# wienkers/marEx

Measured on AMD Instinct MI355X. Metric: Mcells*timesteps/s, shifting_baseline + hobday_extreme p95 (validation+anomaly+thresholds+mask), higher is better.
Workload: dtype f32

## Files before the change

### marex_amd/csrc/marex_common.hip.h

```cpp
#pragma once
#include <hip/hip_runtime.h>

#include <cmath>
#include <type_traits>
#include <cstdarg>
#include <cstdio>
#include <cstring>
#include <map>
#include <string>
#include <vector>

#include "marex_hip.h"

#define NDOY MAREX_NDOY

struct TimedLaunch {
    int kid;
    hipEvent_t a, b;
};

struct marex_ctx {
    int device = 0;
    hipStream_t stream = nullptr;
    std::string err;
    bool timing = false;
    std::vector<TimedLaunch> pending;
    double total_ms[MAREX_K_COUNT] = {0};
    int64_t launches[MAREX_K_COUNT] = {0};
    int* shift_info = nullptr;
    int* shift_plan = nullptr;
    size_t shift_plan_years = 0;
    int* shift_lplan = nullptr;
    size_t shift_lplan_years = 0;
    unsigned char* thr_scratch = nullptr;
    size_t thr_scratch_bytes = 0;
    unsigned char* detrend_scratch = nullptr;
    size_t detrend_scratch_bytes = 0;
    unsigned char* morph_scratch = nullptr;
    size_t morph_scratch_bytes = 0;
    int n_cu = 0;
    std::map<std::string, int> opts;
    long long* row_off = nullptr;
    size_t row_off_bytes = 0;
    long long* row_off_mask = nullptr;
    size_t row_off_mask_bytes = 0;
    unsigned long long* dbg_counters = nullptr;
};

#define MAREX_DBG_COUNTERS 8

static inline int ctx_opt(marex_ctx* ctx, const char* name, int dflt) {
    auto it = ctx->opts.find(name);
    return it == ctx->opts.end() ? dflt : it->second;
}

#ifdef MAREX_ABLATION
#define MAREX_ABLATE_OPT(ctx, name) ctx_opt(ctx, name, 0)
#else
#define MAREX_ABLATE_OPT(ctx, name) 0
#endif

static inline unsigned long long* ctx_debug_counters(marex_ctx* ctx) {
    if (!ctx->dbg_counters) {
        if (hipMalloc((void**)&ctx->dbg_counters, MAREX_DBG_COUNTERS * sizeof(unsigned long long)) != hipSuccess) return nullptr;
        (void)hipMemsetAsync(ctx->dbg_counters, 0, MAREX_DBG_COUNTERS * sizeof(unsigned long long), ctx->stream);
    }
    return ctx->dbg_counters;
}

static inline int device_cus(marex_ctx* ctx) {
    if (ctx->n_cu <= 0) {
        int n = 0;
        if (hipDeviceGetAttribute(&n, hipDeviceAttributeMultiprocessorCount, ctx->device) != hipSuccess || n <= 0) n = 256;
        ctx->n_cu = n;
    }
    return ctx->n_cu;
}

static inline int fail(marex_ctx* ctx, int code, const char* fmt, ...) {
    char buf[512];
    va_list ap;
    va_start(ap, fmt);
    vsnprintf(buf, sizeof buf, fmt, ap);
    va_end(ap);
    if (ctx) ctx->err = buf;
    return code;
}

#define HIP_TRY(ctx, expr)                                                                      \
    do {                                                                                        \
        hipError_t e__ = (expr);                                                                \
        if (e__ != hipSuccess) return fail(ctx, -2, "%s failed: %s", #expr, hipGetErrorString(e__)); \
    } while (0)

struct LaunchTimer {
    marex_ctx* ctx;
    int kid;
    hipEvent_t a = nullptr, b = nullptr;
    LaunchTimer(marex_ctx* c, int k) : ctx(c), kid(k) {
        if (ctx->timing) {
            (void)hipEventCreate(&a);
            (void)hipEventCreate(&b);
            (void)hipEventRecord(a, ctx->stream);
        }
    }
    ~LaunchTimer() {
        if (ctx->timing) {
            (void)hipEventRecord(b, ctx->stream);
            ctx->pending.push_back({kid, a, b});
        }
    }
};

static inline void drain_timers(marex_ctx* ctx) {
    for (auto& p : ctx->pending) {
        float ms = 0.f;
// ... 97 lines not shown
```

### marex_amd/csrc/marex_context.hip

```cpp
#include "marex_common.hip.h"

extern "C" int marex_abi_version(void) { return MAREX_ABI_VERSION; }

extern "C" int marex_workspace_bytes(const marex_workspace_cfg* cfg, size_t* bytes) {
    if (!cfg || !bytes || cfg->T <= 0 || cfg->T_out <= 0 || cfg->T_out > cfg->T || cfg->C <= 0) return -1;
    const size_t C = (size_t)cfg->C, To = (size_t)cfg->T_out;
    for (int i = 0; i < MAREX_WS_COUNT; ++i) bytes[i] = 0;
    bytes[MAREX_WS_ANOMALY] = To * C * sizeof(float);
    bytes[MAREX_WS_EXTREME] = To * C;
    bytes[MAREX_WS_THRESHOLDS] = (size_t)MAREX_NDOY * C * sizeof(float);
    if (cfg->list_rows > 0) {
        const int nper = marex_tail_lists(cfg->max_bucket, cfg->list_rows);
        if (nper < 1) return -1;
        const size_t nch = cfg->list_rows <= 16 ? 2 : 4;
        bytes[MAREX_WS_LISTS] = (size_t)MAREX_NDOY * (size_t)nper * nch * C * 16;
        bytes[MAREX_WS_AUX] = (size_t)MAREX_NDOY * C * sizeof(uint32_t);
    } else {
        bytes[MAREX_WS_BINS] = ((C + 15) / 16) * To * 16 * sizeof(uint16_t);
    }
    bytes[MAREX_WS_PER_CELL] = C * (sizeof(uint8_t) + sizeof(int32_t));
    bytes[MAREX_WS_TOTAL] = bytes[MAREX_WS_ANOMALY] + bytes[MAREX_WS_EXTREME] + 2 * bytes[MAREX_WS_THRESHOLDS] + bytes[MAREX_WS_LISTS] +
                            bytes[MAREX_WS_AUX] + bytes[MAREX_WS_BINS] + bytes[MAREX_WS_PER_CELL];
    return 0;
}

extern "C" int marex_create(int device, marex_ctx** out) {
    if (!out) return -1;
    int n = 0;
    if (hipGetDeviceCount(&n) != hipSuccess || device < 0 || device >= n) return -3;
    marex_ctx* c = new marex_ctx();
    c->device = device;
    extern char** environ;
    for (char** e = environ; e && *e; ++e) {
        if (strncmp(*e, "MAREX_", 6) != 0) continue;
        const char* eq = strchr(*e, '=');
        if (!eq || eq == *e + 6) continue;
        char* end = nullptr;
        const long v = strtol(eq + 1, &end, 10);
        if (end == eq + 1 || *end != '\0') continue;
        c->opts[std::string(*e + 6, (size_t)(eq - (*e + 6)))] = (int)v;
    }
    *out = c;
    return 0;
}

extern "C" int marex_set_option(marex_ctx* ctx, const char* name, int value) {
    if (!ctx || !name || !*name) return -1;
    ctx->opts[name] = value;
    return 0;
}

extern "C" int marex_clear_option(marex_ctx* ctx, const char* name) {
    if (!ctx) return -1;
    if (!name)
        ctx->opts.clear();
    else
        ctx->opts.erase(name);
    return 0;
}

extern "C" int marex_debug_counters(marex_ctx* ctx, uint64_t* out, int reset) {
    if (!ctx || !out) return -1;
    HIP_TRY(ctx, hipSetDevice(ctx->device));
    unsigned long long* d = ctx_debug_counters(ctx);
    if (!d) return fail(ctx, -2, "marex_debug_counters: allocation failed");
    HIP_TRY(ctx, hipStreamSynchronize(ctx->stream));
    HIP_TRY(ctx, hipMemcpy(out, d, MAREX_DBG_COUNTERS * sizeof(unsigned long long), hipMemcpyDeviceToHost));
    if (reset) HIP_TRY(ctx, hipMemsetAsync(d, 0, MAREX_DBG_COUNTERS * sizeof(unsigned long long), ctx->stream));
    return 0;
}

extern "C" int marex_destroy(marex_ctx* ctx) {
    if (!ctx) return -1;
    drain_timers(ctx);
    if (ctx->shift_info) (void)hipFree(ctx->shift_info);
    if (ctx->shift_plan) (void)hipFree(ctx->shift_plan);
    if (ctx->shift_lplan) (void)hipFree(ctx->shift_lplan);
    if (ctx->thr_scratch) (void)hipFree(ctx->thr_scratch);
    if (ctx->detrend_scratch) (void)hipFree(ctx->detrend_scratch);
    if (ctx->morph_scratch) (void)hipFree(ctx->morph_scratch);
    if (ctx->dbg_counters) (void)hipFree(ctx->dbg_counters);
    if (ctx->row_off) (void)hipFree(ctx->row_off);
    if (ctx->row_off_mask) (void)hipFree(ctx->row_off_mask);
    delete ctx;
    return 0;
}

extern "C" const char* marex_last_error(marex_ctx* ctx) { return ctx ? ctx->err.c_str() : "null context"; }

extern "C" int marex_set_stream(marex_ctx* ctx, void* s) {
    if (!ctx) return -1;
    ctx->stream = (hipStream_t)s;
    return 0;
}

extern "C" int marex_sync(marex_ctx* ctx) {
    if (!ctx) return -1;
    HIP_TRY(ctx, hipSetDevice(ctx->device));
    HIP_TRY(ctx, hipStreamSynchronize(ctx->stream));
    drain_timers(ctx);
    return 0;
}

extern "C" int marex_timing_enable(marex_ctx* ctx, int on) {
    if (!ctx) return -1;
    ctx->timing = on != 0;
    return 0;
}

extern "C" int marex_timing_reset(marex_ctx* ctx) {
    if (!ctx) return -1;
    drain_timers(ctx);
    memset(ctx->total_ms, 0, sizeof ctx->total_ms);
    memset(ctx->launches, 0, sizeof ctx->launches);
    return 0;
}

extern "C" int marex_timing_get(marex_ctx* ctx, int kid, double* total_ms, int64_t* launches) {
    if (!ctx || kid < 0 || kid >= MAREX_K_COUNT) return -1;
    drain_timers(ctx);
    if (total_ms) *total_ms = ctx->total_ms[kid];
    if (launches) *launches = ctx->launches[kid];
    return 0;
}
```

### marex_amd/csrc/marex_shifting.hip

```cpp
#include "marex_common.hip.h"
#include "marex_tails.hip.h"
#include <numeric>
#include <utility>

template <int D, int SCAP, bool SEXACT, int WCAP, bool RREG>
__global__ void __launch_bounds__(256)
k_shifting(const float* __restrict__ x, long T, long C, const int4* __restrict__ year_plan, int n_cal, int W,
           int S_rt, int write_clim, const float* __restrict__ edges, int nb, long T_out, float* __restrict__ out,
           unsigned short* __restrict__ bins, unsigned char* __restrict__ mask, int* __restrict__ invalid_count,
           int ncb, int nchunks, int ablate, const int* __restrict__ skip) {
    extern __shared__ float lds[];
#ifndef MAREX_ABLATION
    ablate = 0;
#endif
    float* ring = lds;
    float rr[RREG ? D : 1][RREG ? WCAP : 1];
    const int npad = WCAP - W;
    int4* lplan = reinterpret_cast<int4*>(lds + (RREG ? (size_t)0 : (size_t)D * WCAP * 256));
    float* e = reinterpret_cast<float*>(lplan + (size_t)n_cal * D);

    int cb, chunk;
    if (!xcd_swizzle(blockIdx.x, ncb, nchunks, cb, chunk)) return;
    if (D == 4 && skip && skip[chunk]) return;
    const int tid = threadIdx.x;
// ... 245 lines not shown
}
__device__ __forceinline__ v2f splat2(float v) { return (v2f){v, v}; }

__device__ __forceinline__ v2f div_const2(v2f a, float b, float y) {
    const v2f q = a * splat2(y);
    const v2f r = __builtin_elementwise_fma(-q, splat2(b), a);
    const v2f q2 = __builtin_elementwise_fma(r, splat2(y), q);
    return (v2f){__builtin_amdgcn_div_fixupf(q2.x, b, a.x), __builtin_amdgcn_div_fixupf(q2.y, b, a.y)};
}

typedef __amdgpu_buffer_rsrc_t rsrc_t;
__device__ __forceinline__ rsrc_t make_rsrc(const void* base) {
    return __builtin_amdgcn_make_buffer_rsrc(const_cast<void*>(base), 0, -1, 0x00020000);
}
__device__ __forceinline__ float ldb_f32(rsrc_t r, unsigned voff, int soff) {
    return __builtin_bit_cast(float, __builtin_amdgcn_raw_buffer_load_b32(r, (int)voff, soff, 0));
}
#ifndef ST_AUX_F32
#define ST_AUX_F32 2
#endif
#ifndef ST_AUX_U16
#define ST_AUX_U16 0
#endif
__device__ __forceinline__ void stb_f32(rsrc_t r, unsigned voff, int soff, float v) {
    __builtin_amdgcn_raw_buffer_store_b32(__builtin_bit_cast(unsigned, v), r, (int)voff, soff, ST_AUX_F32);
}
__device__ __forceinline__ void stb_u16(rsrc_t r, unsigned voff, int soff, int v) {
    __builtin_amdgcn_raw_buffer_store_b16((unsigned short)v, r, (int)voff, soff, ST_AUX_U16);
}

typedef int tl_out_rsrc_t __attribute__((ext_vector_type(4)));
__device__ __forceinline__ tl_out_rsrc_t tl_out_make_rsrc(const void* base) {
    const unsigned long long b = (unsigned long long)base;
    tl_out_rsrc_t r;
    r.x = __builtin_amdgcn_readfirstlane((int)(unsigned)b);
    r.y = __builtin_amdgcn_readfirstlane((int)((unsigned)(b >> 32) & 0xFFFFu));
    r.z = -1;
    r.w = 0x00020000;
    return r;
}
__device__ __forceinline__ void tl_out_store(tl_out_rsrc_t r, unsigned voff, unsigned soff, const unsigned (&w)[4]) {
    typedef unsigned u4 __attribute__((ext_vector_type(4)));
    const u4 v = {w[0], w[1], w[2], w[3]};
    const int soff_u = __builtin_amdgcn_readfirstlane((int)soff);
    asm volatile("buffer_store_dwordx4 %0, %1, %2, %3 offen nt\n\ts_nop 2" : : "v"(v), "v"(voff), "s"(r), "s"(soff_u) : "memory");
}


template <int RPW>
struct DmaRows;
#define MAREX_DMA_X4(m, so) "s_mov_b32 m0, " m "\n\ts_nop 0\n\tbuffer_load_dwordx4 %1, %3, " so " offen lds\n\t"
#define MAREX_DMA_X1(m, so) "s_mov_b32 m0, " m "\n\ts_nop 0\n\tbuffer_load_dword %2, %3, " so " offen lds\n\t"
template <>
struct DmaRows<9> {
    static constexpr int NL = 3;
    static __device__ __forceinline__ void issue(tl_out_rsrc_t r, unsigned voff4, unsigned voff1, unsigned l0, unsigned lstep, unsigned so0, unsigned rowb) {
        unsigned keep;
        const unsigned l1 = l0 + 4 * lstep, l2 = l0 + 8 * lstep, so1 = so0 + 4 * rowb, so2 = so0 + 8 * rowb;
        asm volatile("s_mov_b32 %0, m0\n\t" MAREX_DMA_X4("%4", "%7") MAREX_DMA_X4("%5", "%8") MAREX_DMA_X1("%6", "%9") "s_mov_b32 m0, %0"
                     : "=&s"(keep) : "v"(voff4), "v"(voff1), "s"(r), "s"(l0), "s"(l1), "s"(l2), "s"(so0), "s"(so1), "s"(so2) : "memory");
    }
};
template <>
struct DmaRows<8> {
    static constexpr int NL = 2;
    static __device__ __forceinline__ void issue(tl_out_rsrc_t r, unsigned voff4, unsigned voff1, unsigned l0, unsigned lstep, unsigned so0, unsigned rowb) {
        unsigned keep;
        const unsigned l1 = l0 + 4 * lstep, so1 = so0 + 4 * rowb;
        asm volatile("s_mov_b32 %0, m0\n\t" MAREX_DMA_X4("%4", "%6") MAREX_DMA_X4("%5", "%7") "s_mov_b32 m0, %0"
                     : "=&s"(keep) : "v"(voff4), "v"(voff1), "s"(r), "s"(l0), "s"(l1), "s"(so0), "s"(so1) : "memory");
    }
};
template <>
struct DmaRows<7> {
    static constexpr int NL = 4;
    static __device__ __forceinline__ void issue(tl_out_rsrc_t r, unsigned voff4, unsigned voff1, unsigned l0, unsigned lstep, unsigned so0, unsigned rowb) {
        unsigned keep;
        const unsigned l1 = l0 + 4 * lstep, l2 = l0 + 5 * lstep, l3 = l0 + 6 * lstep;
        const unsigned so1 = so0 + 4 * rowb, so2 = so0 + 5 * rowb, so3 = so0 + 6 * rowb;
        asm volatile("s_mov_b32 %0, m0\n\t" MAREX_DMA_X4("%4", "%8") MAREX_DMA_X1("%5", "%9") MAREX_DMA_X1("%6", "%10") MAREX_DMA_X1("%7", "%11") "s_mov_b32 m0, %0"
                     : "=&s"(keep) : "v"(voff4), "v"(voff1), "s"(r), "s"(l0), "s"(l1), "s"(l2), "s"(l3), "s"(so0), "s"(so1), "s"(so2), "s"(so3) : "memory");
    }
};
#undef MAREX_DMA_X4
#undef MAREX_DMA_X1

#define SHIFT_INFO_WORDS 128
#define CLASSIFY_SPLIT 11
#define LEAN_CHUNKS 96

__global__ void k_shift_classify(const int4* __restrict__ year_plan, int n_cal, const float* __restrict__ edges, int nb,
                                 int want_bins, int enable, int* __restrict__ info, int4* __restrict__ fplan, long T, long C,
                                 int reg_S, int4* __restrict__ lplan, const int* __restrict__ doy_start, int wpb, int lean_bins) {
    __shared__ int s_edges_ok;
    const int t = threadIdx.x;
    int eok = 1;
    if (want_bins) {
        const float first = edges[1], delta = edges[2] - edges[1];
        for (int j = 1 + t; j <= nb; j += (int)blockDim.x)
            eok = eok && __float_as_uint(edges[j]) == __float_as_uint(arange_edge(j, first, delta));
    }
    eok = __syncthreads_and(eok);
    if (t == 0) {
        int ok = eok;
        if (want_bins) {
            const float first = edges[1], delta = edges[2] - edges[1], last = edges[nb];
            ok = ok && delta > 0.f && nb < 32768;
            const double m = fabs((double)first) > fabs((double)last) ? fabs((double)first) : fabs((double)last);
            ok = ok && ((double)nb + 2.0 * m / (double)delta) * (1.0 / 1048576.0) < 1.0 / 256.0;
        }
        s_edges_ok = ok && enable;
        info[92] = s_edges_ok;
    }
    __shared__ int s_ok[92];
    if (t < 92) s_ok[t] = 1;
    __syncthreads();
    const int chunk = t / CLASSIFY_SPLIT, sub = t % CLASSIFY_SPLIT;
    if (chunk < 92) {
        const int d0 = chunk * 4;
        int ok = 1;
        for (int y = sub; y < n_cal; y += CLASSIFY_SPLIT) {
            int4 e[4];
            for (int i = 0; i < 4; ++i)
                e[i] = (d0 + i < NDOY) ? year_plan[(size_t)y * NDOY + d0 + i] : make_int4(-1, -1, -1, 0);
            int m = 0;
            while (m < 4 && e[m].x >= 0) ++m;
            if (fplan) {
                const int yn = y + 1 < n_cal ? y + 1 : n_cal - 1;
                const int tbw = year_plan[(size_t)yn * NDOY + (chunk >> 2) * 16].x;
                fplan[((size_t)y * 92 + chunk) * 2] = make_int4(e[0].x, e[0].y, m, e[0].z);
                fplan[((size_t)y * 92 + chunk) * 2 + 1] = make_int4(e[1].z, e[2].z, e[3].z, tbw);
            }
            for (int i = m; i < 4; ++i) ok = ok && e[i].x < 0;
            for (int i = 1; i < m; ++i) {
                ok = ok && e[i].x == e[0].x + i;
                if (e[0].y >= 0)
                    ok = ok && e[i].y == e[0].y + i && e[i].z >= 0;
                else
                    ok = ok && e[i].y < 0;
            }
            if (m > 0 && e[0].y >= 0) ok = ok && e[0].z >= 0;
        }
        if (!ok) atomicAnd(&s_ok[chunk], 0);
    }
    __syncthreads();
    if (chunk < 92 && lplan && reg_S > 0) {
        const int H = reg_S / 2, NPAIR = (reg_S + 3) / 2, NROWS = wpb * ((reg_S + 4 * wpb - 1 + wpb - 1) / wpb);
        const int d0 = chunk * 4, blk16 = (chunk / wpb) * wpb * 4;
        int D1 = 0, D2 = 0, D3 = 0;
        if (lean_bins && d0 + 3 < NDOY)
            for (int y2 = 0; y2 < n_cal; ++y2) {
                const int z0 = year_plan[(size_t)y2 * NDOY + d0].z, z1 = year_plan[(size_t)y2 * NDOY + d0 + 1].z;
                const int z2 = year_plan[(size_t)y2 * NDOY + d0 + 2].z, z3 = year_plan[(size_t)y2 * NDOY + d0 + 3].z;
                if (z0 >= 0 && z1 >= 0 && z2 >= 0 && z3 >= 0) {
                    D1 = z1 - z0;
                    D2 = z2 - z0;
                    D3 = z3 - z0;
                    break;
                }
            }
        for (int yy = sub - 1; yy <= n_cal; yy += CLASSIFY_SPLIT) {
            int flags = 0, tbv = -1, pos = 0;
            long long xoff = 0, ooff = 0;
            if (yy + 1 >= 0 && yy + 1 < n_cal) {
                const int tbn = year_plan[(size_t)(yy + 1) * NDOY + blk16].x;
                if (tbn >= H && (long)tbn - H + NROWS <= T) {
// ... 380 lines not shown
                        stb_u16(rbins, bin_lane, pA.w * 32, k0);
                        if (has1) stb_u16(rbins, bin_lane, pB.x * 32, k1);
                        if (has2) stb_u16(rbins, bin_lane, pB.y * 32, k2);
                        if (has3) stb_u16(rbins, bin_lane, pB.z * 32, k3);
                    }
                }
            }
        }
        rA[J + W] = smA;
        rB[J + W] = smB;
        SSTAMP(tsC);
        if (DMA) {
            if (stage_next) {
                if (dma_pf)
                    asm volatile("s_waitcnt vmcnt(%0)" ::"n"(DmaRows<RPW>::NL) : "memory");
                else
                    asm volatile("s_waitcnt vmcnt(0)" ::: "memory");
            }
            if (o_n > 0 && active) {
                const rsrc_t ro = make_rsrc(out + (size_t)pA.y * C);
                stb_f32(ro, voff, 0, oA.x);
                if (o_n > 1) stb_f32(ro, voff, rowb, oA.y);
                if (o_n > 2) stb_f32(ro, voff, 2 * rowb, oB.x);
                if (o_n > 3) stb_f32(ro, voff, 3 * rowb, oB.y);
            }
            asm volatile("s_barrier" ::: "memory");
        } else {
        if (stage_next) stage_store((y + 1) & 1, nx);
        if (!(SHIFT_EXP & 1)) __syncthreads();
        }
#ifdef SHIFT_STAMPS
        const unsigned long long tsD = __builtin_amdgcn_s_memtime();
        st_top += tsB - tsA;
        st_mid += tsC - tsB;
        st_end += tsD - tsC;
#endif
    };
    for (int y = 0; y < n_cal; y += 2) {
        one_year(y, std::integral_constant<int, 0>{});
        if (TAILS && t_slot == SHIFT_LIST) tails_flush();
        if (y + 1 < n_cal) one_year(y + 1, std::integral_constant<int, 1>{});
        if (TAILS && t_slot == SHIFT_LIST) tails_flush();
#pragma unroll
        for (int j = 0; j < W; ++j) {
            rA[j] = rA[j + 2];
            rB[j] = rB[j + 2];
        }
    }
    if (TAILS && mine) {
        if (t_slot > 0) tails_flush();
        while (t_list < tails.nper) tails_flush();
        if (active) {
            const unsigned cn[4] = {t_cntA & 0xFFFFu, t_cntA >> 16, t_cntB & 0xFFFFu, t_cntB >> 16};
            const unsigned ov[4] = {t_ovfA & 0xFFFFu, t_ovfA >> 16, t_ovfB & 0xFFFFu, t_ovfB >> 16};
#pragma unroll
            for (int di = 0; di < 4; ++di)
                if (d0 + di < NDOY) tails.aux[(size_t)(d0 + di) * C + c] = tail_aux_word(cn[di], ov[di]);
        }
    }
    if (invalid_count && active && n_invalid) atomicAdd(&invalid_count[c], n_invalid);
#ifdef SHIFT_STAMPS
    if (TAILS && lane == 0 && tails.dbg) {
        atomicAdd(&tails.dbg[5], st_top);
        atomicAdd(&tails.dbg[6], st_mid);
        atomicAdd(&tails.dbg[7], st_end);
        atomicAdd(&tails.dbg[4], 1ull);
    }
#endif
}

template <typename F, int... Is>
__device__ __forceinline__ void unroll_steps_impl(F& f, std::integer_sequence<int, Is...>) {
    (f(std::integral_constant<int, Is>{}), ...);
}
template <int N, typename F>
__device__ __forceinline__ void unroll_steps(F&& f) {
    unroll_steps_impl(f, std::make_integer_sequence<int, N>{});
}

#define LR_REG 1
#define LR_OUT 2
#define LR_STAGE_NEXT 4

template <int W, int S, int NWV, bool BINS>
__global__ void __launch_bounds__(64 * NWV, 16 / NWV)
k_shift_lean(const float* __restrict__ x, int T, int C, const int4* __restrict__ fplan, const int4* __restrict__ lplan, int n_cal,
             const int* __restrict__ info, const float* __restrict__ edges, int nb, float* __restrict__ out,
             unsigned char* __restrict__ mask, int* __restrict__ invalid_count, int ncg, int nblk, TailOut tails,
             unsigned short* __restrict__ bins, long T_out) {
    int cg, bc;
    if (!xcd_swizzle(blockIdx.x, ncg, nblk, cg, bc)) return;
    const int wave = __builtin_amdgcn_readfirstlane((int)(threadIdx.x >> 6));
    const int lane = (int)(threadIdx.x & 63);
    const int chunk = bc * NWV + wave;
    static_assert((S & 1) == 1 && S >= 5 && S <= 25, "k_shift_lean: odd smoothing widths 5..25");
    static_assert(NWV == 4 || NWV == 8, "k_shift_lean: 4 or 8 waves");
    constexpr int H = S / 2, NPAIR = (S + 3) / 2, NST = S + 4 * NWV - 1, RPW = (NST + NWV - 1) / NWV;
    constexpr int NROWS = NWV * RPW;
    __shared__ float stage[NROWS * 64];
    __shared__ unsigned newkeys[BINS ? 1 : NWV][2][BINS ? 1 : SHIFT_LIST][64];
    const bool mine = chunk < 92 && info[chunk] != 0;
    const int d0 = mine ? chunk * 4 : 0;
    const int c = cg * 64 + lane;
    const bool active = c < C;
    const unsigned cidx = active ? (unsigned)c : (unsigned)(C - 1);
    const unsigned voff = cidx * 4u;
    const int rowb = C * 4;
    const float e_first = edges[1], e_delta = edges[2] - edges[1], e_last = edges[nb];
    const float inv_width = (float)(nb - 1) / (e_last - e_first);
    constexpr float Sf = (float)S;
    const float yS = 1.0f / Sf;
    const float Wf = (float)W;
    const float yW = 1.0f / Wf;
    const float nbm1f = (float)(nb - 1);
    const float c0 = (1.0f - e_first * inv_width) - 0.0078125f;
    const float qnan = nan_f();
    if (chunk == 0 && mine && mask && active) mask[c] = finite_f(x[c]) ? 1 : 0;
    const unsigned bin_lane = (((cidx >> 4) - (unsigned)(cg * 4)) * (unsigned)T_out * 16u + (cidx & 15u)) * 2u;
    const rsrc_t rbins = make_rsrc(BINS ? bins + (size_t)(cg * 4) * (size_t)T_out * 16 : nullptr);
    int bD1 = 0, bD2 = 0, bD3 = 0;

    typedef __attribute__((address_space(3))) float lds_f32;
    const int c4 = cg * 64 + (lane & 15) * 4;
    const unsigned dma_voff4 = (unsigned)(lane >> 4) * (unsigned)rowb + (unsigned)(c4 + 4 <= C ? c4 : C - 4) * 4u;
    const unsigned dma_lds = (unsigned)__builtin_amdgcn_readfirstlane((int)(unsigned)(size_t)(lds_f32*)&stage[(RPW * wave) * 64]);
    const char* xw = reinterpret_cast<const char*>(x) + (size_t)(RPW * wave) * (size_t)C * 4;
    auto dma_rows = [&](int lo, int hi) __attribute__((always_inline)) {
        const unsigned long long off = ((unsigned long long)(unsigned)hi << 32) | (unsigned)lo;
        DmaRows<RPW>::issue(tl_out_make_rsrc(xw + off), dma_voff4, voff, dma_lds, 256u, 0u, (unsigned)rowb);
    };
    constexpr int LSTRIDE = LEAN_CHUNKS * 2;
    const int4* lr_next = lplan + (size_t)chunk * 2;
    {
        const int4 pre = lr_next[0];
        if (BINS) {
            const int4 preB = lr_next[1];
            bD1 = preB.y;
            bD2 = preB.z;
            bD3 = preB.w;
        }
        if (pre.x & LR_STAGE_NEXT) {
            dma_rows(pre.z, pre.w);
            asm volatile("s_waitcnt vmcnt(0)" ::: "memory");
        }
        asm volatile("s_barrier" ::: "memory");
        lr_next += LSTRIDE;
    }
    int4 nA = lr_next[0], nB = lr_next[1];
    lr_next += LSTRIDE;

    constexpr int U = W >= 13 ? 3 : 2;
    v2f hA[W + U], hB[W + U];
#pragma unroll
    for (int j = 0; j < W + U; ++j) hA[j] = hB[j] = splat2(qnan);
    int n_invalid = 0;
    unsigned t_cntA = 0, t_cntB = 0, t_ovfA = 0, t_ovfB = 0;
    int t_slot = 0, t_list = 0;
    int n_lean = 0, n_gen = 0;
    auto tails_flush = [&]() __attribute__((always_inline)) {
        const tl_out_rsrc_t rl = tl_out_make_rsrc(tails.lists + (size_t)d0 * tails.nper * 2 * (size_t)C);
        const unsigned lvoff = cidx * 16u;
#pragma unroll
        for (int pr = 0; pr < 2; ++pr) {
            unsigned v[16];
#pragma unroll
            for (int u = 0; u < 16; ++u) v[u] = (u < SHIFT_LIST && u < t_slot) ? newkeys[wave][pr][u][lane] : 0u;
            sort16_desc(v);
#pragma unroll
            for (int h = 0; h < 2; ++h) {
                const int di = 2 * pr + h;
                if (d0 + di < NDOY) {
#pragma unroll
                    for (int jj = 0; jj < 2; ++jj) {
                        unsigned w[4];
#pragma unroll
                        for (int i = 0; i < 4; ++i) {
                            const unsigned a = v[8 * jj + 2 * i], b = v[8 * jj + 2 * i + 1];
                            w[i] = h == 0 ? ((a & 0xFFFFu) | (b << 16)) : ((a >> 16) | (b & 0xFFFF0000u));
                        }
                        const int li = __builtin_amdgcn_readfirstlane((di * tails.nper + t_list) * 2 + jj);
                        if (active) tl_out_store(rl, lvoff, (unsigned)li * (unsigned)C * 16u, w);
                    }
                }
            }
        }
        ++t_list;
        t_slot = 0;
    };

    auto mid = [&](const int4& cA) __attribute__((always_inline)) {
        asm volatile("s_waitcnt lgkmcnt(0)\n\ts_barrier" ::: "memory");
        if (cA.x & LR_STAGE_NEXT) dma_rows(cA.z, cA.w);
        nA = lr_next[0];
        nB = lr_next[1];
        lr_next += LSTRIDE;
    };
    constexpr int NH0 = (NPAIR + 1) / 2, NH1 = NPAIR - NH0;
    static_assert(NH0 >= 2, "the second chain starts in the first half");
    v2f xh[NH0];
    v2f accA = splat2(0.f), accB = splat2(0.f);
    float xc0 = 0.f, xc1 = 0.f, xc2 = 0.f, xc3 = 0.f;
    auto load_half = [&](auto Pc, int how, int ts) __attribute__((always_inline)) {
        constexpr int P = decltype(Pc)::value, M0 = P ? NH0 : 0, MN = P ? NH1 : NH0;
        if (how == 0) {
            const float* st = &stage[(4 * wave) * 64 + lane];
#pragma unroll
            for (int m = 0; m < MN; ++m) {
                xh[m].x = st[(2 * (M0 + m)) * 64];
                xh[m].y = st[(2 * (M0 + m) + 1) * 64];
            }
        } else if (how == 1) {
            const rsrc_t rx = make_rsrc(x + (size_t)(ts - H) * (size_t)C);
#pragma unroll
            for (int m = 0; m < MN; ++m) {
                xh[m].x = ldb_f32(rx, voff, (2 * (M0 + m)) * rowb);
                xh[m].y = ldb_f32(rx, voff, (2 * (M0 + m) + 1) * rowb);
            }
        } else {
#pragma unroll
            for (int m = 0; m < MN; ++m) {
                int ra = ts - H + 2 * (M0 + m), rb = ra + 1;
                ra = ra < 0 ? 0 : (ra > T - 1 ? T - 1 : ra);
                rb = rb < 0 ? 0 : (rb > T - 1 ? T - 1 : rb);
                xh[m].x = ldb_f32(make_rsrc(x + (size_t)ra * (size_t)C), voff, 0);
                xh[m].y = ldb_f32(make_rsrc(x + (size_t)rb * (size_t)C), voff, 0);
            }
        }
    };
    auto half = [&](auto Pc) __attribute__((always_inline)) {
        constexpr int P = decltype(Pc)::value, M0 = P ? NH0 : 0, M1 = P ? NPAIR : NH0;
        if constexpr (S == 21) {
#define PK_LO(acc, src) "v_pk_add_f32 %" #acc ", %" #acc ", %" #src " op_sel_hi:[1,0]\n\t"
#define PK_HI(acc, src) "v_pk_add_f32 %" #acc ", %" #acc ", %" #src " op_sel:[0,1] op_sel_hi:[1,1]\n\t"
#define PK_BOTH(src) PK_LO(0, src) PK_LO(1, src) PK_HI(0, src) PK_HI(1, src)
            if (P == 0) {
                accA = (v2f){xh[0].x, -0.0f};
                accB = (v2f){xh[1].x, -0.0f};
                asm(PK_HI(0, 2) PK_LO(0, 3) PK_HI(0, 3) PK_HI(1, 3) PK_BOTH(4) PK_BOTH(5) PK_BOTH(6) PK_BOTH(7)
                    : "+v"(accA), "+v"(accB)
                    : "v"(xh[0]), "v"(xh[1]), "v"(xh[2]), "v"(xh[3]), "v"(xh[4]), "v"(xh[5]));
                xc0 = xh[5].x;
                xc1 = xh[5].y;
            } else {
                asm(PK_BOTH(2) PK_BOTH(3) PK_BOTH(4) PK_BOTH(5) PK_LO(0, 6) PK_LO(1, 6) PK_HI(1, 6) PK_LO(1, 7)
                    : "+v"(accA), "+v"(accB)
                    : "v"(xh[0]), "v"(xh[1]), "v"(xh[2]), "v"(xh[3]), "v"(xh[4]), "v"(xh[5]));
                accA.y += xh[4].y;
                accB.y += xh[5].y;
                xc2 = xh[0].x;
                xc3 = xh[0].y;
            }
#undef PK_BOTH
#undef PK_HI
#undef PK_LO
            return;
        }
        if (P == 0) accA = (v2f){xh[0].x, -0.0f};
#pragma unroll
        for (int s = 1; s <= S - 1; ++s)
            if ((s >> 1) >= M0 && (s >> 1) < M1) accA = (s & 1) ? pk_add_bc_hi(accA, xh[(s >> 1) - M0]) : pk_add_bc_lo(accA, xh[(s >> 1) - M0]);
        if ((S >> 1) >= M0 && (S >> 1) < M1) accA.y += xh[(S >> 1) - M0].y;
        if (1 >= M0 && 1 < M1) accB = (v2f){xh[1 - M0].x, -0.0f};
#pragma unroll
        for (int s = 3; s <= S + 1; ++s)
            if ((s >> 1) >= M0 && (s >> 1) < M1) accB = (s & 1) ? pk_add_bc_hi(accB, xh[(s >> 1) - M0]) : pk_add_bc_lo(accB, xh[(s >> 1) - M0]);
        if (((S + 2) >> 1) >= M0 && ((S + 2) >> 1) < M1) accB.y += xh[((S + 2) >> 1) - M0].y;
#define MAREX_XC(i, dst) \
    if (((H + i) >> 1) >= M0 && ((H + i) >> 1) < M1) dst = ((H + i) & 1) ? xh[((H + i) >> 1) - M0].y : xh[((H + i) >> 1) - M0].x;
        MAREX_XC(0, xc0) MAREX_XC(1, xc1) MAREX_XC(2, xc2) MAREX_XC(3, xc3)
#undef MAREX_XC
    };
    auto smooth = [&](const int4& cA, v2f& smA, v2f& smB, v2f& xcA, v2f& xcB, int how, int ts) __attribute__((always_inline)) {
        load_half(std::integral_constant<int, 0>{}, how, ts);
        half(std::integral_constant<int, 0>{});
        load_half(std::integral_constant<int, 1>{}, how, ts);
// ... 165 lines not shown
            const bool staged = tb >= H && tb - H + NROWS <= T && pA.x == tb + 4 * wave;
            v2f xcA, xcB;
            smooth(cA, smA, smB, xcA, xcB, staged ? 0 : (edge ? 2 : 1), pA.x);
            if (edge) {
                const int t0 = pA.x;
                smA.x = (t0 - H >= 0 && t0 + H < T) ? smA.x : qnan;
                smA.y = (t0 + 1 - H >= 0 && t0 + 1 + H < T) ? smA.y : qnan;
                smB.x = (t0 + 2 - H >= 0 && t0 + 2 + H < T) ? smB.x : qnan;
                smB.y = (t0 + 3 - H >= 0 && t0 + 3 + H < T) ? smB.y : qnan;
            }
            const bool has1 = nd > 1, has2 = nd > 2, has3 = nd > 3;
            n_invalid += finite_f(xcA.x) ? 0 : 1;
            if (has1) n_invalid += finite_f(xcA.y) ? 0 : 1; else smA.y = qnan;
            if (has2) n_invalid += finite_f(xcB.x) ? 0 : 1; else smB.x = qnan;
            if (has3) n_invalid += finite_f(xcB.y) ? 0 : 1; else smB.y = qnan;
            asm volatile("s_waitcnt vmcnt(0)" ::: "memory");
            if (pA.y >= 0) {
                v2f aA, aB;
                anomaly(Jc, xcA, xcB, aA, aB);
                const rsrc_t ro = make_rsrc(out + (size_t)pA.y * (size_t)C);
                if (active) {
                    stb_f32(ro, voff, 0, aA.x);
                    if (has1) stb_f32(ro, voff, rowb, aA.y);
                    if (has2) stb_f32(ro, voff, 2 * rowb, aB.x);
                    if (has3) stb_f32(ro, voff, 3 * rowb, aB.y);
                }
                int k0, k1, k2, k3;
                digit2(aA, k0, k1);
                digit2(aB, k2, k3);
                if constexpr (BINS) {
                    if (active) {
                        stb_u16(rbins, bin_lane, pA.w * 32, (aA.x == aA.x) ? k0 : nb);
                        if (has1) stb_u16(rbins, bin_lane, pB.x * 32, (aA.y == aA.y) ? k1 : nb);
                        if (has2) stb_u16(rbins, bin_lane, pB.y * 32, (aB.x == aB.x) ? k2 : nb);
                        if (has3) stb_u16(rbins, bin_lane, pB.z * 32, (aB.y == aB.y) ? k3 : nb);
                    }
                } else {
                const float l1 = has1 ? e_last : -__builtin_inff(), l2 = has2 ? e_last : -__builtin_inff(),
                            l3 = has3 ? e_last : -__builtin_inff();
                const bool v0 = aA.x < e_last, v1 = aA.y < l1, v2 = aB.x < l2, v3 = aB.y < l3;
                const int ds0 = tails.doy_start[d0], ds1 = tails.doy_start[d0 + 1 < NDOY ? d0 + 1 : NDOY - 1];
                const int ds2 = tails.doy_start[d0 + 2 < NDOY ? d0 + 2 : NDOY - 1], ds3 = tails.doy_start[d0 + 3 < NDOY ? d0 + 3 : NDOY - 1];
                const unsigned p0 = (unsigned)(pA.w - ds0), p1 = (unsigned)(pB.x - ds1), p2 = (unsigned)(pB.y - ds2), p3 = (unsigned)(pB.z - ds3);
                const unsigned q0 = v0 ? ((unsigned)k0 << TAIL_POS_BITS) + 128u + p0 : 0u, q1 = v1 ? ((unsigned)k1 << TAIL_POS_BITS) + 128u + p1 : 0u;
                const unsigned q2 = v2 ? ((unsigned)k2 << TAIL_POS_BITS) + 128u + p2 : 0u, q3 = v3 ? ((unsigned)k3 << TAIL_POS_BITS) + 128u + p3 : 0u;
                newkeys[wave][0][t_slot][lane] = q0 | (q1 << 16);
                newkeys[wave][1][t_slot][lane] = q2 | (q3 << 16);
                t_cntA += (v0 ? 1u : 0u) + (v1 ? 0x10000u : 0u);
                t_cntB += (v2 ? 1u : 0u) + (v3 ? 0x10000u : 0u);
                const float mx = fmaxf(fmaxf(aA.x, has1 ? aA.y : aA.x), fmaxf(has2 ? aB.x : aA.x, has3 ? aB.y : aA.x));
                if (__builtin_amdgcn_ballot_w64(mx >= e_last) != 0) {
                    unsigned s0 = t_ovfA & 0xFFFFu, s1 = t_ovfA >> 16, s2 = t_ovfB & 0xFFFFu, s3 = t_ovfB >> 16;
                    if (aA.x >= e_last) s0 = tail_ovf_add(s0, p0);
                    if (has1 && aA.y >= e_last) s1 = tail_ovf_add(s1, p1);
                    if (has2 && aB.x >= e_last) s2 = tail_ovf_add(s2, p2);
                    if (has3 && aB.y >= e_last) s3 = tail_ovf_add(s3, p3);
                    t_ovfA = s0 | (s1 << 16);
                    t_ovfB = s2 | (s3 << 16);
                }
                ++t_slot;
                }
            }
        } else {
            mid(cA);
            asm volatile("s_waitcnt vmcnt(0)" ::: "memory");
        }
        hA[J + W] = smA;
        hB[J + W] = smB;
    };

#define MAREX_LEAN_YEAR(J, yy)                                                                                  \
    {                                                                                                           \
        const int4 cA = nA, cB = nB;                                                                            \
        if (mine && (cA.x & LR_REG)) {                                                                          \
            lean_year(std::integral_constant<int, J>{}, cA, cB);                                                \
            ++n_lean;                                                                                           \
        } else {                                                                                                \
            general_year(std::integral_constant<int, J>{}, yy, cA);                                             \
            n_gen += mine ? 1 : 0;                                                                              \
        }                                                                                                       \
        asm volatile("s_barrier" ::: "memory");  \
        if (!BINS && t_slot == SHIFT_LIST) tails_flush();                                                       \
    }
    for (int y = 0; y < n_cal; y += U) {
        MAREX_LEAN_YEAR(0, y)
        if constexpr (U > 1) if (y + 1 < n_cal) MAREX_LEAN_YEAR(1, y + 1)
        if constexpr (U > 2) if (y + 2 < n_cal) MAREX_LEAN_YEAR(2, y + 2)
        if constexpr (U > 3) if (y + 3 < n_cal) MAREX_LEAN_YEAR(3, y + 3)
#pragma unroll
        for (int j = 0; j < W; ++j) {
            hA[j] = hA[j + U];
            hB[j] = hB[j + U];
        }
    }
#undef MAREX_LEAN_YEAR
    if (mine && !BINS) {
        if (t_slot > 0) tails_flush();
        while (t_list < tails.nper) tails_flush();
        if (active) {
            const unsigned cn[4] = {t_cntA & 0xFFFFu, t_cntA >> 16, t_cntB & 0xFFFFu, t_cntB >> 16};
            const unsigned ov[4] = {t_ovfA & 0xFFFFu, t_ovfA >> 16, t_ovfB & 0xFFFFu, t_ovfB >> 16};
#pragma unroll
            for (int di = 0; di < 4; ++di)
                if (d0 + di < NDOY) tails.aux[(size_t)(d0 + di) * (size_t)C + c] = tail_aux_word(cn[di], ov[di]);
        }
    }
    if (invalid_count && active && n_invalid) atomicAdd(&invalid_count[c], n_invalid);
#ifdef MAREX_LEAN_COUNTERS
    if (tails.dbg && lane == 0) {
        atomicAdd(&tails.dbg[6], (unsigned long long)n_lean);
        atomicAdd(&tails.dbg[7], (unsigned long long)n_gen);
    }
#endif
}

static bool lean_instance(int W, int S) { return S == 21 && (W == 15 || W == 5); }

struct ShiftArgs {
    const float* x;
    int64_t T, C;
    const int4* year_plan;
    const int4* fplan;
    int n_cal;
    int W, S, write_clim;
    const float* edges;
    int nb;
    int64_t T_out;
    float* out;
    uint16_t* bins;
    uint8_t* mask;
    int32_t* invalid_count;
    const int* skip;
    TailOut tails;
    bool lean = false;
    const int4* lplan = nullptr;
    int lean_waves = 4;
};

template <int D, int SCAP, bool SEXACT, int WCAP, bool RREG>
static int launch_shifting(marex_ctx* ctx, const ShiftArgs& a) {
    const int ncb = (int)((a.C + 255) / 256);
    const int nchunks = (NDOY + D - 1) / D;
    const size_t lds = ((RREG ? (size_t)0 : (size_t)D * WCAP * 256) + (a.bins ? (size_t)a.nb + 1 : 0)) * sizeof(float) + (size_t)a.n_cal * D * 16;
    if (lds > 80 * 1024) return fail(ctx, -4, "marex_shifting_baseline_f32: window_year_baseline=%d needs more than 80 KiB of LDS", a.W);
    auto kern = k_shifting<D, SCAP, SEXACT, WCAP, RREG>;
    if (lds > 48 * 1024)
        HIP_TRY(ctx, hipFuncSetAttribute((const void*)kern, hipFuncAttributeMaxDynamicSharedMemorySize, (int)lds));
    hipLaunchKernelGGL(kern, dim3(xcd_grid(ncb, nchunks)), dim3(256), lds, ctx->stream, a.x, (long)a.T, (long)a.C,
                       a.year_plan, a.n_cal, a.W, a.S, a.write_clim, a.edges, a.nb, (long)a.T_out, a.out, a.bins,
                       a.mask, a.invalid_count, ncb, nchunks, MAREX_ABLATE_OPT(ctx, "SHIFT_ABLATE"), D == 4 ? a.skip : nullptr);
    HIP_TRY(ctx, hipGetLastError());
    return 0;
}

template <int W, int S = 21>
static void launch_shift_fast(marex_ctx* ctx, const ShiftArgs& a) {
    const int ncg = (int)((a.C + 63) / 64);
#define MAREX_SF_ARGS dim3(xcd_grid(ncg, 23)), dim3(256), 0, ctx->stream, a.x, (long)a.T, (long)a.C, a.fplan, a.n_cal, a.skip, a.write_clim, a.edges, a.nb, (long)a.T_out, a.out, a.bins, a.mask, a.invalid_count, ncg, 23, a.tails
    if (a.lean && (a.tails.lists || a.bins)) {
        if constexpr (S == 21 && (W == 15 || W == 5)) {
            if (a.tails.lists)
                hipLaunchKernelGGL((k_shift_lean<W, S, 4, false>), dim3(xcd_grid(ncg, 23)), dim3(256), 0, ctx->stream, a.x, (int)a.T, (int)a.C,
                                   a.fplan, a.lplan, a.n_cal, a.skip, a.edges, a.nb, a.out, a.mask, a.invalid_count, ncg, 23, a.tails,
                                   (unsigned short*)nullptr, (long)a.T_out);
            else
                hipLaunchKernelGGL((k_shift_lean<W, S, 4, true>), dim3(xcd_grid(ncg, 23)), dim3(256), 0, ctx->stream, a.x, (int)a.T, (int)a.C,
                                   a.fplan, a.lplan, a.n_cal, a.skip, a.edges, a.nb, a.out, a.mask, a.invalid_count, ncg, 23, a.tails,
                                   a.bins, (long)a.T_out);
        }
    } else if (a.tails.lists) {
        constexpr int RPW = (S + 15 + 3) / 4;
        constexpr bool has_dma = S == 21 && (W == 15 || W == 5);
        const bool dma = has_dma && ctx_opt(ctx, "SHIFT_DMA", 0) != 0 && a.C >= 4 && a.C % 4 == 0 &&
                         (unsigned long long)(365 + 4 * RPW + 4) * (unsigned long long)a.C * 4ull < 0xFFFFFFFFull;
        if (dma)
            hipLaunchKernelGGL((k_shift_fast<W, true, S, has_dma>), MAREX_SF_ARGS);
        else
            hipLaunchKernelGGL((k_shift_fast<W, true, S, false>), MAREX_SF_ARGS);
    } else {
        hipLaunchKernelGGL((k_shift_fast<W, false, S, false>), MAREX_SF_ARGS);
    }
#undef MAREX_SF_ARGS
}

template <int D, int WCAP, bool RREG>
static int dispatch_shifting_S(marex_ctx* ctx, const ShiftArgs& a) {
    if (a.S == 21) return launch_shifting<D, 21, true, WCAP, RREG>(ctx, a);
    return launch_shifting<D, 1, false, WCAP, RREG>(ctx, a);
}

static int shifting_impl(marex_ctx* ctx, const char* who, const float* x, int64_t T, int64_t C, const int32_t* year_plan,
                         int n_cal_years, int W, int S, int write_clim, const float* edges, int nb, int64_t T_out, float* out,
                         uint16_t* bins, uint8_t* mask, int32_t* invalid_count, TailOut tails, bool* all_fast_possible) {
    if (!ctx) return -1;
    if (!x || !year_plan || !out || T <= 0 || C <= 0 || n_cal_years <= 0)
        return fail(ctx, -1, "%s: null pointer or empty shape", who);
    if (((uintptr_t)year_plan & 15) != 0) return fail(ctx, -1, "%s: year_plan must be 16-byte aligned", who);
    if (W < 1 || S < 1) return fail(ctx, -1, "%s: W and S must be >= 1", who);
    if (S > T) S = (int)T + 1;
    if (W > 64) return fail(ctx, -4, "%s: window_year_baseline > 64 is not supported", who);
    if ((bins || tails.lists) && (!edges || nb < 4 || nb > 65534 || T_out <= 0))
        return fail(ctx, -1, "%s: binning needs edges, T_out and 4 <= nb <= 65534", who);
    HIP_TRY(ctx, hipSetDevice(ctx->device));
    ShiftArgs a{x, T, C, reinterpret_cast<const int4*>(year_plan), nullptr, n_cal_years, W, S, write_clim,
                edges, nb, T_out, out, bins, mask, invalid_count, nullptr, tails};
    const int forceD = ctx_opt(ctx, "SHIFT_D", 0);
    const int reg = ctx_opt(ctx, "SHIFT_RING", 1);
    const bool fast_w = W == 3 || W == 4 || W == 5 || W == 6 || W == 7 || W == 10 || W == 13 || W == 15;
    const bool fast_ws = S == 21 ? fast_w : ((S == 11 || S == 15) && (W == 5 || W == 10 || W == 15));
    const bool fast_cfg = ctx_opt(ctx, "SHIFT_FAST", 1) != 0 && fast_ws && forceD == 0 && T >= S + 3 &&
                          T_out < (1 << 24) && C < (1 << 24) && MAREX_ABLATE_OPT(ctx, "SHIFT_ABLATE") == 0;
    if (all_fast_possible) *all_fast_possible = fast_cfg;
    if (fast_cfg && !ctx->shift_info) HIP_TRY(ctx, hipMalloc((void**)&ctx->shift_info, SHIFT_INFO_WORDS * sizeof(int)));
    if (fast_cfg && ctx->shift_plan_years < (size_t)n_cal_years) {
        if (ctx->shift_plan) {
            HIP_TRY(ctx, hipStreamSynchronize(ctx->stream));
            (void)hipFree(ctx->shift_plan);
            ctx->shift_plan = nullptr;
            ctx->shift_plan_years = 0;
        }
        HIP_TRY(ctx, hipMalloc((void**)&ctx->shift_plan, (size_t)n_cal_years * 92 * 8 * sizeof(int)));
        ctx->shift_plan_years = (size_t)n_cal_years;
    }
    LaunchTimer lt(ctx, MAREX_K_SHIFTING);
    if (fast_cfg) {
        const bool lean_bins = !tails.lists && bins && !write_clim && ctx_opt(ctx, "SHIFT_LEAN_BINS", 1) != 0;
        const bool lean = (tails.lists || lean_bins) && lean_instance(W, S) && ctx_opt(ctx, "SHIFT_LEAN", 1) != 0 && C >= 4 && C % 4 == 0 &&
                          T < (1ll << 31) - 64 && (unsigned long long)(S + 31 + 8 + 4) * (unsigned long long)C * 4ull < 0xFFFFFFFFull;
        const int lean_waves = 4;
        if (lean && ctx->shift_lplan_years < (size_t)n_cal_years) {
            if (ctx->shift_lplan) {
                HIP_TRY(ctx, hipStreamSynchronize(ctx->stream));
                (void)hipFree(ctx->shift_lplan);
                ctx->shift_lplan = nullptr;
                ctx->shift_lplan_years = 0;
            }
            HIP_TRY(ctx, hipMalloc((void**)&ctx->shift_lplan, ((size_t)n_cal_years + 2) * LEAN_CHUNKS * 8 * sizeof(int)));
            ctx->shift_lplan_years = (size_t)n_cal_years;
        }
        hipLaunchKernelGGL(k_shift_classify, dim3(1), dim3(1024), 0, ctx->stream, a.year_plan, n_cal_years, edges, nb,
                           (bins || tails.lists) ? 1 : 0, 1, ctx->shift_info, reinterpret_cast<int4*>(ctx->shift_plan), (long)T, (long)C,
                           lean ? S : 0, lean ? reinterpret_cast<int4*>(ctx->shift_lplan) : nullptr, tails.doy_start, lean_waves,
                           (lean && lean_bins) ? 1 : 0);
        a.lean_waves = lean_waves;
        a.lplan = reinterpret_cast<const int4*>(ctx->shift_lplan);
        a.lean = lean;
        a.skip = ctx->shift_info;
        a.fplan = reinterpret_cast<const int4*>(ctx->shift_plan);
        if (S == 11 || S == 15) {
            switch (W * 100 + S) {
                case 511: launch_shift_fast<5, 11>(ctx, a); break;
                case 515: launch_shift_fast<5, 15>(ctx, a); break;
                case 1011: launch_shift_fast<10, 11>(ctx, a); break;
                case 1015: launch_shift_fast<10, 15>(ctx, a); break;
                case 1511: launch_shift_fast<15, 11>(ctx, a); break;
                default: launch_shift_fast<15, 15>(ctx, a); break;
            }
        } else
        switch (W) {
            case 3: launch_shift_fast<3>(ctx, a); break;
            case 4: launch_shift_fast<4>(ctx, a); break;
            case 5: launch_shift_fast<5>(ctx, a); break;
            case 6: launch_shift_fast<6>(ctx, a); break;
            case 7: launch_shift_fast<7>(ctx, a); break;
            case 10: launch_shift_fast<10>(ctx, a); break;
            case 13: launch_shift_fast<13>(ctx, a); break;
            default: launch_shift_fast<15>(ctx, a); break;
        }
        HIP_TRY(ctx, hipGetLastError());
    }
    if (W <= 8) {
        if (reg) return forceD == 2 ? dispatch_shifting_S<2, 8, true>(ctx, a) : forceD == 8 ? dispatch_shifting_S<8, 8, true>(ctx, a) : dispatch_shifting_S<4, 8, true>(ctx, a);
        return forceD == 1 ? dispatch_shifting_S<1, 8, false>(ctx, a) : dispatch_shifting_S<4, 8, false>(ctx, a);
    }
    if (W <= 16) {
        if (reg) return forceD == 2 ? dispatch_shifting_S<2, 16, true>(ctx, a) : dispatch_shifting_S<4, 16, true>(ctx, a);
        return forceD == 1 ? dispatch_shifting_S<1, 16, false>(ctx, a) : dispatch_shifting_S<4, 16, false>(ctx, a);
    }
    return dispatch_shifting_S<1, 64, false>(ctx, a);
}

extern "C" int marex_shifting_baseline_f32(marex_ctx* ctx, const float* x, int64_t T, int64_t C,
                                           const int32_t* year_plan, int n_cal_years, int W, int S,
                                           int write_clim, const float* edges, int nb, int64_t T_out, float* out,
                                           uint16_t* bins, uint8_t* mask, int32_t* invalid_count) {
    return shifting_impl(ctx, "marex_shifting_baseline_f32", x, T, C, year_plan, n_cal_years, W, S, write_clim, edges, nb, T_out, out,
                         bins, mask, invalid_count, TailOut{nullptr, nullptr, nullptr, 0, nullptr}, nullptr);
}

int marex_tail_extract_impl(marex_ctx* ctx, const float* anom, int64_t T_out, int64_t C, const int32_t* doy_start,
                            const int32_t* doy_rows, int max_bucket, const float* edges, int nb, int list_rows, void* lists,
                            uint32_t* aux, const int* skip_chunks);

extern "C" int marex_shifting_baseline_tails_f32(marex_ctx* ctx, const float* x, int64_t T, int64_t C, const int32_t* year_plan,
                                                 int n_cal_years, int W, int S, const float* edges, int nb, int64_t T_out,
                                                 float* out, uint8_t* mask, int32_t* invalid_count, const int32_t* doy_start,
                                                 const int32_t* doy_rows, int max_bucket, void* lists, uint32_t* aux) {
    if (!ctx) return -1;
    if (!doy_start || !doy_rows || !lists || !aux) return fail(ctx, -1, "marex_shifting_baseline_tails_f32: null pointer");
    if (nb > TAIL_MAX_NB || max_bucket < 1 || max_bucket > 6 * SHIFT_LIST || C > (1 << 24))
        return fail(ctx, -4, "marex_shifting_baseline_tails_f32: shape outside the emitted tail format (nb <= %d, buckets <= %d rows)",
                    TAIL_MAX_NB, 6 * SHIFT_LIST);
    if (((uintptr_t)lists & 15) != 0) return fail(ctx, -1, "marex_shifting_baseline_tails_f32: lists must be 16-byte aligned");
    TailOut t{reinterpret_cast<uint4*>(lists), aux, doy_start, (max_bucket + SHIFT_LIST - 1) / SHIFT_LIST, ctx_debug_counters(ctx)};
    bool fast = false;
    const int rc = shifting_impl(ctx, "marex_shifting_baseline_tails_f32", x, T, C, year_plan, n_cal_years, W, S, 0, edges, nb, T_out,
                                 out, nullptr, mask, invalid_count, t, &fast);
    if (rc != 0) return rc;
    return marex_tail_extract_impl(ctx, out, T_out, C, doy_start, doy_rows, max_bucket, edges, nb, SHIFT_LIST, lists, aux,
                                   fast ? ctx->shift_info : nullptr);
}
```

Baseline: 319,000.

## Pace neighbouring lean shift blocks to keep them in lockstep across years

Adds an on-by-default pacing scheme to the lean shifting kernel. Every few years, wave 0 of each block publishes its year progress to a device buffer and briefly sleeps while a neighbouring block in the same column group falls more than a small lag behind. The goal is to keep adjacent blocks close in time so their overlapping halo rows are still cached when reused. It adds a memset and a pacing buffer allocation, atomic traffic and possible stalls, and the sleep loop has bounded retries. Experimental paths for no-halo DMA and skipping list stores are compiled only under SHIFT_EXP flags.

```diff
diff --git a/marex_amd/csrc/marex_common.hip.h b/marex_amd/csrc/marex_common.hip.h
--- a/marex_amd/csrc/marex_common.hip.h
+++ b/marex_amd/csrc/marex_common.hip.h
@@ -32,6 +32,8 @@
     size_t shift_plan_years = 0;
     int* shift_lplan = nullptr;
     size_t shift_lplan_years = 0;
+    int* shift_pace = nullptr;
+    size_t shift_pace_words = 0;
     unsigned char* thr_scratch = nullptr;
     size_t thr_scratch_bytes = 0;
     unsigned char* detrend_scratch = nullptr;
diff --git a/marex_amd/csrc/marex_context.hip b/marex_amd/csrc/marex_context.hip
--- a/marex_amd/csrc/marex_context.hip
+++ b/marex_amd/csrc/marex_context.hip
@@ -76,6 +76,7 @@
     if (ctx->shift_info) (void)hipFree(ctx->shift_info);
     if (ctx->shift_plan) (void)hipFree(ctx->shift_plan);
     if (ctx->shift_lplan) (void)hipFree(ctx->shift_lplan);
+    if (ctx->shift_pace) (void)hipFree(ctx->shift_pace);
     if (ctx->thr_scratch) (void)hipFree(ctx->thr_scratch);
     if (ctx->detrend_scratch) (void)hipFree(ctx->detrend_scratch);
     if (ctx->morph_scratch) (void)hipFree(ctx->morph_scratch);
diff --git a/marex_amd/csrc/marex_shifting.hip b/marex_amd/csrc/marex_shifting.hip
--- a/marex_amd/csrc/marex_shifting.hip
+++ b/marex_amd/csrc/marex_shifting.hip
@@ -351,6 +351,17 @@
                      : "=&s"(keep) : "v"(voff4), "v"(voff1), "s"(r), "s"(l0), "s"(l1), "s"(l2), "s"(l3), "s"(so0), "s"(so1), "s"(so2), "s"(so3) : "memory");
     }
 };
+#if SHIFT_EXP & 64
+template <>
+struct DmaRows<4> {
+    static constexpr int NL = 1;
+    static __device__ __forceinline__ void issue(tl_out_rsrc_t r, unsigned voff4, unsigned voff1, unsigned l0, unsigned lstep, unsigned so0, unsigned rowb) {
+        unsigned keep;
+        asm volatile("s_mov_b32 %0, m0\n\t" MAREX_DMA_X4("%4", "%5") "s_mov_b32 m0, %0"
+                     : "=&s"(keep) : "v"(voff4), "v"(voff1), "s"(r), "s"(l0), "s"(so0) : "memory");
+    }
+};
+#endif
 #undef MAREX_DMA_X4
 #undef MAREX_DMA_X1
 
@@ -897,12 +908,35 @@
 #define LR_OUT 2
 #define LR_STAGE_NEXT 4
 
+#ifndef SHIFT_PACE_DEFAULT
+#define SHIFT_PACE_DEFAULT 1
+#endif
+#ifndef SHIFT_PACE_K
+#define SHIFT_PACE_K 6
+#endif
+#ifndef SHIFT_PACE_L
+#define SHIFT_PACE_L 2
+#endif
+#ifndef SHIFT_PACE_SLEEP
+#define SHIFT_PACE_SLEEP 16
+#endif
+#ifndef SHIFT_PACE_N
+#define SHIFT_PACE_N 4
+#endif
+#ifndef SHIFT_PACE_B
+#define SHIFT_PACE_B 12
+#endif
+static_assert(SHIFT_PACE_K >= 1 && SHIFT_PACE_L >= 0 && SHIFT_PACE_SLEEP >= 1 && SHIFT_PACE_SLEEP <= 127 && SHIFT_PACE_N >= 1 &&
+              SHIFT_PACE_N <= 64 && SHIFT_PACE_B >= 0 && SHIFT_PACE_B <= 256, "pacing constants: bounded waits only");
+#define PACE_STRIDE 24
+#define PACE_DONE 0x7FFFFFFF
+
 template <int W, int S, int NWV, bool BINS>
 __global__ void __launch_bounds__(64 * NWV, 16 / NWV)
 k_shift_lean(const float* __restrict__ x, int T, int C, const int4* __restrict__ fplan, const int4* __restrict__ lplan, int n_cal,
              const int* __restrict__ info, const float* __restrict__ edges, int nb, float* __restrict__ out,
              unsigned char* __restrict__ mask, int* __restrict__ invalid_count, int ncg, int nblk, TailOut tails,
-             unsigned short* __restrict__ bins, long T_out) {
+             unsigned short* __restrict__ bins, long T_out, int* pace, int exp_nolists) {
     int cg, bc;
     if (!xcd_swizzle(blockIdx.x, ncg, nblk, cg, bc)) return;
     const int wave = __builtin_amdgcn_readfirstlane((int)(threadIdx.x >> 6));
@@ -944,6 +978,17 @@
         const unsigned long long off = ((unsigned long long)(unsigned)hi << 32) | (unsigned)lo;
         DmaRows<RPW>::issue(tl_out_make_rsrc(xw + off), dma_voff4, voff, dma_lds, 256u, 0u, (unsigned)rowb);
     };
+#if SHIFT_EXP & 64
+    static_assert(NWV == 4 && H + 16 <= NROWS, "no-halo experiment: the 16 centre rows lie inside the stage");
+    const unsigned dma_lds_c = (unsigned)__builtin_amdgcn_readfirstlane((int)(unsigned)(size_t)(lds_f32*)&stage[(H + 4 * wave) * 64]);
+    const char* xc = reinterpret_cast<const char*>(x) + (size_t)(H + 4 * wave) * (size_t)C * 4;
+    auto dma_rows_year = [&](int lo, int hi) __attribute__((always_inline)) {
+        const unsigned long long off = ((unsigned long long)(unsigned)hi << 32) | (unsigned)lo;
+        DmaRows<4>::issue(tl_out_make_rsrc(xc + off), dma_voff4, voff, dma_lds_c, 256u, 0u, (unsigned)rowb);
+    };
+#else
+    auto& dma_rows_year = dma_rows;
+#endif
     constexpr int LSTRIDE = LEAN_CHUNKS * 2;
     const int4* lr_next = lplan + (size_t)chunk * 2;
     {
@@ -994,7 +1039,7 @@
                             w[i] = h == 0 ? ((a & 0xFFFFu) | (b << 16)) : ((a >> 16) | (b & 0xFFFF0000u));
                         }
                         const int li = __builtin_amdgcn_readfirstlane((di * tails.nper + t_list) * 2 + jj);
-                        if (active) tl_out_store(rl, lvoff, (unsigned)li * (unsigned)C * 16u, w);
+                        if (active && !((SHIFT_EXP & 128) && exp_nolists)) tl_out_store(rl, lvoff, (unsigned)li * (unsigned)C * 16u, w);
                     }
                 }
             }
@@ -1005,7 +1050,7 @@
 
     auto mid = [&](const int4& cA) __attribute__((always_inline)) {
         asm volatile("s_waitcnt lgkmcnt(0)\n\ts_barrier" ::: "memory");
-        if (cA.x & LR_STAGE_NEXT) dma_rows(cA.z, cA.w);
+        if (cA.x & LR_STAGE_NEXT) dma_rows_year(cA.z, cA.w);
         nA = lr_next[0];
         nB = lr_next[1];
         lr_next += LSTRIDE;
@@ -1337,7 +1382,31 @@
         asm volatile("s_barrier" ::: "memory");  \
         if (!BINS && t_slot == SHIFT_LIST) tails_flush();                                                       \
     }
+    const bool pacing = pace != nullptr && wave == 0;
+    int* const pace_me = pace + (size_t)cg * PACE_STRIDE + bc;
+    const int pace_lo = bc > 0 ? -1 : 0, pace_hi = bc + 1 < nblk ? 1 : 0;
+    int pace_next = 0, pace_left = SHIFT_PACE_B;
     for (int y = 0; y < n_cal; y += U) {
+        if (pacing && y >= pace_next) {
+            pace_next = y + SHIFT_PACE_K;
+            if (lane == 0) __hip_atomic_store(pace_me, y + 1, __ATOMIC_RELAXED, __HIP_MEMORY_SCOPE_AGENT);
+#pragma unroll 1
+            for (int i = 0; i < SHIFT_PACE_N; ++i) {
+                int a = 0, b = 0;
+                if (lane == 0) {
+                    a = __hip_atomic_load(pace_me + pace_lo, __ATOMIC_RELAXED, __HIP_MEMORY_SCOPE_AGENT);
+                    b = __hip_atomic_load(pace_me + pace_hi, __ATOMIC_RELAXED, __HIP_MEMORY_SCOPE_AGENT);
+                }
+                a = __builtin_amdgcn_readfirstlane(a);
+                b = __builtin_amdgcn_readfirstlane(b);
+                a = (a > 0 && a != PACE_DONE) ? a : PACE_DONE;
+                b = (b > 0 && b != PACE_DONE) ? b : PACE_DONE;
+                const int slow = a < b ? a : b;
+                if (pace_left <= 0 || slow == PACE_DONE || y + 1 - slow <= SHIFT_PACE_L) break;
+                --pace_left;
+                __builtin_amdgcn_s_sleep(SHIFT_PACE_SLEEP);
+            }
+        }
         MAREX_LEAN_YEAR(0, y)
         if constexpr (U > 1) if (y + 1 < n_cal) MAREX_LEAN_YEAR(1, y + 1)
         if constexpr (U > 2) if (y + 2 < n_cal) MAREX_LEAN_YEAR(2, y + 2)
@@ -1349,6 +1418,7 @@
         }
     }
 #undef MAREX_LEAN_YEAR
+    if (pacing && lane == 0) __hip_atomic_store(pace_me, PACE_DONE, __ATOMIC_RELAXED, __HIP_MEMORY_SCOPE_AGENT);
     if (mine && !BINS) {
         if (t_slot > 0) tails_flush();
         while (t_list < tails.nper) tails_flush();
@@ -1390,6 +1460,8 @@
     bool lean = false;
     const int4* lplan = nullptr;
     int lean_waves = 4;
+    int* pace = nullptr;
+    int exp_nolists = 0;
 };
 
 template <int D, int SCAP, bool SEXACT, int WCAP, bool RREG>
@@ -1417,11 +1489,11 @@
             if (a.tails.lists)
                 hipLaunchKernelGGL((k_shift_lean<W, S, 4, false>), dim3(xcd_grid(ncg, 23)), dim3(256), 0, ctx->stream, a.x, (int)a.T, (int)a.C,
                                    a.fplan, a.lplan, a.n_cal, a.skip, a.edges, a.nb, a.out, a.mask, a.invalid_count, ncg, 23, a.tails,
-                                   (unsigned short*)nullptr, (long)a.T_out);
+                                   (unsigned short*)nullptr, (long)a.T_out, a.pace, a.exp_nolists);
             else
                 hipLaunchKernelGGL((k_shift_lean<W, S, 4, true>), dim3(xcd_grid(ncg, 23)), dim3(256), 0, ctx->stream, a.x, (int)a.T, (int)a.C,
                                    a.fplan, a.lplan, a.n_cal, a.skip, a.edges, a.nb, a.out, a.mask, a.invalid_count, ncg, 23, a.tails,
-                                   a.bins, (long)a.T_out);
+                                   a.bins, (long)a.T_out, a.pace, a.exp_nolists);
         }
     } else if (a.tails.lists) {
         constexpr int RPW = (S + 15 + 3) / 4;
@@ -1493,6 +1565,27 @@
             HIP_TRY(ctx, hipMalloc((void**)&ctx->shift_lplan, ((size_t)n_cal_years + 2) * LEAN_CHUNKS * 8 * sizeof(int)));
             ctx->shift_lplan_years = (size_t)n_cal_years;
         }
+        if (lean && ctx_opt(ctx, "SHIFT_PACE", SHIFT_PACE_DEFAULT) != 0) {
+            const size_t words = (size_t)xcd_grid((int)((C + 63) / 64), PACE_STRIDE);
+            if (ctx->shift_pace_words < words) {
+                if (ctx->shift_pace) {
+                    HIP_TRY(ctx, hipStreamSynchronize(ctx->stream));
+                    (void)hipFree(ctx->shift_pace);
+                    ctx->shift_pace = nullptr;
+                    ctx->shift_pace_words = 0;
+                }
+                HIP_TRY(ctx, hipMalloc((void**)&ctx->shift_pace, words * sizeof(int)));
+                ctx->shift_pace_words = words;
+            }
+            HIP_TRY(ctx, hipMemsetAsync(ctx->shift_pace, 0, words * sizeof(int), ctx->stream));
+            a.pace = ctx->shift_pace;
+        }
+#if SHIFT_EXP & 128
+        if (lean) {
+            static std::map<marex_ctx*, int> lean_launches;
+            a.exp_nolists = ++lean_launches[ctx] >= ctx_opt(ctx, "SHIFT_EXP_NOLISTS_FROM", 1 << 30) ? 1 : 0;
+        }
+#endif
         hipLaunchKernelGGL(k_shift_classify, dim3(1), dim3(1024), 0, ctx->stream, a.year_plan, n_cal_years, edges, nb,
                            (bins || tails.lists) ? 1 : 0, 1, ctx->shift_info, reinterpret_cast<int4*>(ctx->shift_plan), (long)T, (long)C,
                            lean ? S : 0, lean ? reinterpret_cast<int4*>(ctx->shift_lplan) : nullptr, tails.doy_start, lean_waves,
```

Result: slower. 300,400, median of 2 (-5.8%).
